# RViMLab/ECCV2022-multi-scale-and-cross-scale-contrastive-segmentation

Hardware: NVIDIA B200
Metric: ms+cs contrastive loss fwd+bwd anchor-pairs/s (higher is better)
Workload: dtype bf16

## Files before the change

### eccv2022-multi-scale-and-cross-scale-contrastive-segmentation_b200/csrc/common.cuh

```cuda
#pragma once
#include <cuda_runtime.h>
#include <cuda_bf16.h>
#include <cuda_fp16.h>
#include <stdint.h>
#include <stdio.h>
#include <stdarg.h>

#include "../../include/mscs.h"

namespace mscs {

void set_error(const char* fmt, ...);
const char* get_error();

#define MSCS_CHECK_ARG(cond, ...)                                   \
  do {                                                              \
    if (!(cond)) { ::mscs::set_error(__VA_ARGS__); return -1; }     \
  } while (0)

#define MSCS_CUDA(expr)                                                                   \
  do {                                                                                    \
    cudaError_t _e = (expr);                                                              \
    if (_e != cudaSuccess) {                                                              \
      ::mscs::set_error("%s failed: %s (%s:%d)", #expr, cudaGetErrorString(_e), __FILE__, \
// ... 31 lines not shown
  cfg.numAttrs = pdl_enabled() ? 1 : 0;
  return cudaLaunchKernelEx(&cfg, kernel, static_cast<P>(args)...);
}

__device__ __forceinline__ float warp_sum(float v) {
#pragma unroll
  for (int o = 16; o > 0; o >>= 1) v += __shfl_xor_sync(0xffffffffu, v, o);
  return v;
}

__device__ __forceinline__ float to_f32(float x) { return x; }
__device__ __forceinline__ float to_f32(__nv_bfloat16 x) { return __bfloat162float(x); }
__device__ __forceinline__ float to_f32(__half x) { return __half2float(x); }
template <typename T> __device__ __forceinline__ T from_f32(float x);
template <> __device__ __forceinline__ float from_f32<float>(float x) { return x; }
template <> __device__ __forceinline__ __nv_bfloat16 from_f32<__nv_bfloat16>(float x) { return __float2bfloat16_rn(x); }
template <> __device__ __forceinline__ __half from_f32<__half>(float x) { return __float2half_rn(x); }

__device__ __forceinline__ uint32_t pack2(__nv_bfloat16*, float a, float b) {
  const __nv_bfloat162 h = __floats2bfloat162_rn(a, b);
  return reinterpret_cast<const uint32_t&>(h);
}
__device__ __forceinline__ uint32_t pack2(__half*, float a, float b) {
  const __half2 h = __floats2half2_rn(a, b);
  return reinterpret_cast<const uint32_t&>(h);
}

__device__ __forceinline__ void st16_cs(float* p, const float (&v)[4]) {
  __stcs(reinterpret_cast<float4*>(p), make_float4(v[0], v[1], v[2], v[3]));
}
template <typename T>
__device__ __forceinline__ void st16_cs(T* p, const float (&v)[8]) {
  const uint4 u = make_uint4(pack2(p, v[0], v[1]), pack2(p, v[2], v[3]), pack2(p, v[4], v[5]), pack2(p, v[6], v[7]));
  __stcs(reinterpret_cast<uint4*>(p), u);
}

__device__ __forceinline__ void ld4(const float* p, float (&v)[4]) {
  const float4 x = *reinterpret_cast<const float4*>(p);
  v[0] = x.x; v[1] = x.y; v[2] = x.z; v[3] = x.w;
}
template <typename T>
__device__ __forceinline__ void ld4(const T* p, float (&v)[4]) {
  const uint2 u = *reinterpret_cast<const uint2*>(p);
  const T* h = reinterpret_cast<const T*>(&u);
#pragma unroll
  for (int q = 0; q < 4; ++q) v[q] = to_f32(h[q]);
}
__device__ __forceinline__ void st4_cs(float* p, const float (&v)[4]) { st16_cs(p, v); }
template <typename T>
__device__ __forceinline__ void st4_cs(T* p, const float (&v)[4]) {
  __stcs(reinterpret_cast<uint2*>(p), make_uint2(pack2(p, v[0], v[1]), pack2(p, v[2], v[3])));
}

static inline int dtype_bytes(int dtype) {
  return dtype == MSCS_DTYPE_F32 ? 4 : (dtype == MSCS_DTYPE_BF16 || dtype == MSCS_DTYPE_F16) ? 2 : 0;
}

}
```

### eccv2022-multi-scale-and-cross-scale-contrastive-segmentation_b200/csrc/gather.cu

```cuda
#include "common.cuh"

namespace mscs {

constexpr int kMaxC = 256;

__global__ void __launch_bounds__(256)
k_gather_normalize(const float* __restrict__ feat, int C, int C_pad, int plane, const int* __restrict__ pix,
                   int N, int N_pad, __nv_bfloat16* __restrict__ anc_bf16, float* __restrict__ anc_f32,
                   float* __restrict__ inv_norm) {
  pdl_trigger();
  const int lane = threadIdx.x & 31;
  const int row = blockIdx.x * (blockDim.x >> 5) + (threadIdx.x >> 5);
  if (row >= N_pad) return;
  __nv_bfloat16* orow = anc_bf16 + (size_t)row * C_pad;
  if (row >= N) {
    for (int c = lane; c < C_pad; c += 32) orow[c] = __float2bfloat16(0.f);
    return;
  }
  const int gp = pix[row];
  if (gp < 0) {
    for (int c = lane; c < C_pad; c += 32) orow[c] = __float2bfloat16(0.f);
    return;
  }
  const int b = gp / plane, p = gp - b * plane;
// ... 286 lines not shown

template <typename T>
__global__ void __launch_bounds__(256) k_scatter_rows_nhwc(const __grid_constant__ RowsBatch g) {
  int s = 0;
  while (s + 1 < g.count && (int)blockIdx.x >= g.block0[s + 1]) ++s;
  const int lane = threadIdx.x & 31;
  const int row = ((int)blockIdx.x - g.block0[s]) * 8 + (threadIdx.x >> 5);
  if (row >= g.rows[s] || (g.n_rows_dev[s] && row >= *g.n_rows_dev[s])) return;
  const int gp = g.pix[s][row];
  if (gp < 0) return;
  const int C = g.C[s];
  const float* gr = g.dF[s] + (size_t)row * g.ldF[s];
  const float* f = g.f32[s] + (size_t)row * C;
  float gv[kMaxC / 32], fv[kMaxC / 32], dot = 0.f;
#pragma unroll
  for (int q = 0; q < kMaxC / 32; ++q) {
    const int c = lane + 32 * q;
    gv[q] = (c < C) ? gr[c] : 0.f;
    fv[q] = (c < C) ? f[c] : 0.f;
    dot = fmaf(gv[q], fv[q], dot);
  }
  dot = warp_sum(dot);
  const float inv = g.inv[s][row];
  const bool clamped = inv >= 1e12f;
  T* dst = static_cast<T*>(g.dfeat[s]) + (size_t)gp * C;
#pragma unroll
  for (int q = 0; q < kMaxC / 32; ++q) {
    const int c = lane + 32 * q;
    if (c < C) dst[c] = from_f32<T>((clamped ? gv[q] : (gv[q] - fv[q] * dot)) * inv);
  }
}

template <typename T, bool GATHER>
__global__ void __launch_bounds__(256) k_rows_raw_nhwc(const __grid_constant__ RowsBatch g) {
  int s = 0;
  while (s + 1 < g.count && (int)blockIdx.x >= g.block0[s + 1]) ++s;
  const int lane = threadIdx.x & 31;
  const int row = ((int)blockIdx.x - g.block0[s]) * 8 + (threadIdx.x >> 5);
  if (row >= g.rows[s] || (g.n_rows_dev[s] && row >= *g.n_rows_dev[s])) return;
  const int gp = g.pix[s][row];
  if (gp < 0) return;
  const int C = g.C[s];
  if (GATHER) {
    const T* src = static_cast<const T*>(g.feat[s]) + (size_t)gp * C;
    float* dst = g.f32[s] + (size_t)row * C;
    for (int c = lane; c < C; c += 32) dst[c] = to_f32(__ldg(src + c));
  } else {
    const float* src = g.dF[s] + (size_t)row * g.ldF[s];
    T* dst = static_cast<T*>(g.dfeat[s]) + (size_t)gp * C;
    for (int c = lane; c < C; c += 32) dst[c] = from_f32<T>(src[c]);
  }
}

struct DenseStream {
  const float* dx[MSCS_MAX_SCALES]; const int* slot[MSCS_MAX_SCALES]; void* dfeat[MSCS_MAX_SCALES];
  int ld[MSCS_MAX_SCALES], C[MSCS_MAX_SCALES], plane[MSCS_MAX_SCALES], npix[MSCS_MAX_SCALES], blk0[MSCS_MAX_SCALES + 1];
  int count;
};
template <typename T>
__global__ void __launch_bounds__(128) k_dense_stream(const __grid_constant__ DenseStream g) {
  constexpr int P = 16 / sizeof(T);
  int s = 0;
  while (s + 1 < g.count && (int)blockIdx.x >= g.blk0[s + 1]) ++s;
  const int lin = (((int)blockIdx.x - g.blk0[s]) * 128 + (int)threadIdx.x) * P;
  if (lin >= g.npix[s]) return;
  const int plane = g.plane[s], C = g.C[s], ld = g.ld[s];
  int sl[P];
#pragma unroll
  for (int i = 0; i < P; i += 4) {
    const int4 q = *reinterpret_cast<const int4*>(g.slot[s] + lin + i);
    sl[i] = q.x; sl[i + 1] = q.y; sl[i + 2] = q.z; sl[i + 3] = q.w;
  }
  const int b = lin / plane, p = lin - b * plane;
  T* __restrict__ out = static_cast<T*>(g.dfeat[s]) + ((size_t)b * C) * plane + p;
  const float* __restrict__ dx = g.dx[s];
  const float* r[P];
  bool h[P];
#pragma unroll
  for (int i = 0; i < P; ++i) { r[i] = dx + (size_t)max(sl[i], 0) * ld; h[i] = sl[i] >= 0; }
#pragma unroll 8
  for (int c = 0; c < C; ++c) {
    float v[P];
#pragma unroll
    for (int i = 0; i < P; ++i) v[i] = h[i] ? __ldg(r[i] + c) : 0.f;
    st16_cs(out + (size_t)c * plane, v);
  }
}

}

using namespace mscs;

extern "C" int mscs_gather_normalize_sectors(const float* feat, int n, int C, int plane, const int32_t* slot, int N,
                                             void* anc_bf16, float* anc_f32, float* inv_norm, void* stream_) {
  MSCS_CHECK_ARG(feat && slot && anc_bf16 && anc_f32 && inv_norm, "null pointer argument");
  MSCS_CHECK_ARG(C >= 1 && C <= kMaxC, "C=%d unsupported (1..%d)", C, kMaxC);
  MSCS_CHECK_ARG(n >= 1 && plane >= 8 && plane % 8 == 0 && N >= 1, "bad sizes (plane must be a multiple of 8)");
  cudaStream_t st = (cudaStream_t)stream_;
  const int C_pad = (C + 63) / 64 * 64, N_pad = (N + 255) / 256 * 256;
  if (N_pad > N)
    MSCS_CUDA(cudaMemsetAsync((__nv_bfloat16*)anc_bf16 + (size_t)N * C_pad, 0,
                              sizeof(__nv_bfloat16) * (size_t)(N_pad - N) * C_pad, st));
  const int n_oct = n * (plane / 8);
  k_gather_sectors<<<ceil_div(n_oct, 8), 256, 0, st>>>(feat, C, C_pad, plane, slot, n_oct, (__nv_bfloat16*)anc_bf16,
                                                       anc_f32, inv_norm, nullptr);
  MSCS_LAUNCH_CHECK();
  return 0;
}

extern "C" int mscs_slot_map(const int32_t* pix, int N, int n_pixels, int32_t* slot, void* stream_) {
  MSCS_CHECK_ARG(pix && slot && N >= 1 && n_pixels >= 1, "bad arguments");
  cudaStream_t st = (cudaStream_t)stream_;
  MSCS_CUDA(cudaMemsetAsync(slot, 0xff, sizeof(int) * (size_t)n_pixels, st));
  k_slot_map<<<ceil_div(N, 256), 256, 0, st>>>(pix, N, slot);
  MSCS_LAUNCH_CHECK();
  return 0;
}

extern "C" int mscs_scatter_sectors_pull(void* const* slabs, int world, size_t dF_byte_off, int rows_per_rank, int ldF,
                                         const float* anc_f32, const float* inv_norm, const int32_t* slot, int n, int C,
                                         int plane, float* dfeat, void* stream_) {
  MSCS_CHECK_ARG(slabs && anc_f32 && inv_norm && slot && dfeat, "null pointer argument");
  MSCS_CHECK_ARG(world >= 1 && world <= MSCS_MAX_RANKS && rows_per_rank >= 1, "bad world %d / rows per rank %d", world,
                 rows_per_rank);
  MSCS_CHECK_ARG(C >= 1 && C <= kMaxC && ldF >= C, "C=%d / ldF=%d unsupported", C, ldF);
  MSCS_CHECK_ARG(plane % 8 == 0, "plane %d is not a multiple of 8 pixels", plane);
  PullRows pull{};
  pull.n = world; pull.rows_per_rank = rows_per_rank;
  for (int r = 0; r < world; ++r) {
    MSCS_CHECK_ARG(slabs[r] != nullptr, "peer %d: null slab pointer", r);
    pull.p[r] = reinterpret_cast<const float*>((const char*)slabs[r] + dF_byte_off);
  }
  const int n_oct = n * (plane / 8);
  k_scatter_sectors_pull<<<ceil_div(n_oct, 8), 256, 0, (cudaStream_t)stream_>>>(pull, ldF, anc_f32, inv_norm, slot,
// ... 76 lines not shown
  scatter_sectors_body(g.dF[s], g.ldF[s], g.f32[s], g.inv[s], g.slot[s], g.n_oct[s], g.C[s], g.plane[s], g.dfeat[s],
                       g.block0[s]);
}

extern "C" int mscs_scatter_sectors_batch(const mscs_scatter_item* items, int count, void* stream_) {
  MSCS_CHECK_ARG(items && count >= 1 && count <= MSCS_MAX_SCALES, "bad item count %d", count);
  ScatterBatch g{};
  g.count = count;
  int blocks = 0;
  for (int s = 0; s < count; ++s) {
    const mscs_scatter_item& it = items[s];
    MSCS_CHECK_ARG(it.dF && it.anc_f32 && it.inv_norm && it.slot && it.dfeat, "item %d: null pointer argument", s);
    MSCS_CHECK_ARG(it.C >= 1 && it.C <= kMaxC && it.ldF >= it.C, "item %d: C=%d / ldF=%d unsupported", s, it.C, it.ldF);
    MSCS_CHECK_ARG(it.plane % 8 == 0, "item %d: plane %d is not a multiple of 8 pixels", s, it.plane);
    if (int rc = check_dtype(s, it.dtype, it.dfeat, 16, "dfeat")) return rc;
    MSCS_CHECK_ARG(it.dtype == MSCS_DTYPE_F32, "item %d: the sector scatter writes fp32 gradients only", s);
    g.dF[s] = it.dF; g.f32[s] = it.anc_f32; g.inv[s] = it.inv_norm; g.slot[s] = it.slot; g.dfeat[s] = (float*)it.dfeat;
    g.ldF[s] = it.ldF; g.C[s] = it.C; g.plane[s] = it.plane; g.n_oct[s] = it.n * (it.plane / 8);
    g.block0[s] = blocks;
    blocks += ceil_div(g.n_oct[s], 8);
  }
  g.block0[count] = blocks;
  k_scatter_sectors_batch<<<blocks, 256, 0, (cudaStream_t)stream_>>>(g);
  MSCS_LAUNCH_CHECK();
  return 0;
}


extern "C" int mscs_gather_normalize(const float* feat, int n, int C, int plane, const int32_t* pix, int N,
                                     void* anc_bf16, float* anc_f32, float* inv_norm, void* stream_) {
  MSCS_CHECK_ARG(feat && pix && anc_bf16 && anc_f32 && inv_norm, "null pointer argument");
  MSCS_CHECK_ARG(C >= 1 && C <= kMaxC, "C=%d unsupported (1..%d)", C, kMaxC);
  MSCS_CHECK_ARG(n >= 1 && plane >= 1 && N >= 1, "bad sizes");
  const int C_pad = (C + 63) / 64 * 64, N_pad = (N + 255) / 256 * 256;
  k_gather_normalize<<<ceil_div(N_pad, 8), 256, 0, (cudaStream_t)stream_>>>(
      feat, C, C_pad, plane, pix, N, N_pad, (__nv_bfloat16*)anc_bf16, anc_f32, inv_norm);
  MSCS_LAUNCH_CHECK();
  return 0;
}

extern "C" int mscs_scatter_grad(const float* dF, int ldF, const float* anc_f32, const float* inv_norm,
                                 const int32_t* pix, int N, int n, int C, int plane, float* dfeat,
                                 int zero_fill, void* stream_) {
  MSCS_CHECK_ARG(dF && anc_f32 && inv_norm && pix && dfeat, "null pointer argument");
  MSCS_CHECK_ARG(C >= 1 && C <= kMaxC && ldF >= C, "C=%d / ldF=%d unsupported", C, ldF);
  cudaStream_t st = (cudaStream_t)stream_;
  if (zero_fill) MSCS_CUDA(cudaMemsetAsync(dfeat, 0, sizeof(float) * (size_t)n * C * plane, st));
  k_scatter_grad<<<ceil_div(N, 8), 256, 0, st>>>(dF, ldF, anc_f32, inv_norm, pix, N, C, plane, dfeat);
  MSCS_LAUNCH_CHECK();
  return 0;
}

template <typename T>
static int dense_stream_launch(const DenseBatch& g, const mscs_scatter_item* items, int dtype, cudaStream_t st) {
  DenseStream d{};
  int blk = 0;
  for (int s = 0; s < g.count; ++s) {
    if (items[s].dtype != dtype) continue;
    const int j = d.count++;
    d.dx[j] = g.dF[s]; d.slot[j] = g.slot[s]; d.dfeat[j] = items[s].dfeat; d.ld[j] = g.ldF[s]; d.C[j] = g.C[s];
    d.plane[j] = g.plane[s]; d.npix[j] = g.n[s] * g.plane[s]; d.blk0[j] = blk;
    blk += ceil_div(d.npix[j], 128 * (16 / (int)sizeof(T)));
  }
  if (d.count == 0) return 0;
  d.blk0[d.count] = blk;
  k_dense_stream<T><<<blk, 128, 0, st>>>(d);
  MSCS_LAUNCH_CHECK();
  return 0;
}

extern "C" int mscs_scatter_dense_batch(const mscs_scatter_item* items, const int32_t* rows, int count, void* stream_) {
  MSCS_CHECK_ARG(items && rows && count >= 1 && count <= MSCS_MAX_SCALES, "bad arguments");
  DenseBatch g{};
  g.count = count;
  int rb = 0, n_raw = 0;
  for (int s = 0; s < count; ++s) {
    const mscs_scatter_item& it = items[s];
    MSCS_CHECK_ARG(it.dF && it.slot && it.dfeat, "item %d: null pointer argument", s);
    MSCS_CHECK_ARG((it.anc_f32 == nullptr) == (it.inv_norm == nullptr),
                   "item %d: anc_f32 and inv_norm must both be set or both be NULL (raw rows)", s);
    const bool raw = it.anc_f32 == nullptr;
    n_raw += raw;
    MSCS_CHECK_ARG(it.C >= 1 && it.C <= kMaxC && it.ldF >= it.C, "item %d: C=%d / ldF=%d unsupported", s, it.C, it.ldF);
    MSCS_CHECK_ARG(it.plane % 4 == 0 && rows[s] >= 0, "item %d: plane %d is not a multiple of 4 pixels", s, it.plane);
    if (int rc = check_dtype(s, it.dtype, it.dfeat, 16, "dfeat")) return rc;
    MSCS_CHECK_ARG(it.dtype == MSCS_DTYPE_F32 || it.plane % 8 == 0,
                   "item %d: half gradients need a plane that is a multiple of 8 pixels (plane %d)", s, it.plane);
    g.dF[s] = const_cast<float*>(it.dF); g.f32[s] = it.anc_f32; g.inv[s] = it.inv_norm; g.slot[s] = it.slot;
    g.ldF[s] = it.ldF; g.C[s] = it.C; g.plane[s] = it.plane; g.n[s] = it.n; g.rows[s] = raw ? 0 : rows[s];
    g.n_rows_dev[s] = it.n_rows_dev;
    MSCS_CHECK_ARG((long long)it.n * it.C * it.plane < (1ll << 32), "item %d: more than 2^32 gradient elements", s);
    g.rowblk0[s] = rb; rb += ceil_div(g.rows[s], 8);
  }
  g.rowblk0[count] = rb;
  cudaStream_t st = (cudaStream_t)stream_;
  if (n_raw < count) {
    k_dx_rows<<<rb > 0 ? rb : 1, 256, 0, st>>>(g);
    MSCS_LAUNCH_CHECK();
  }
  if (int rc = dense_stream_launch<float>(g, items, MSCS_DTYPE_F32, st)) return rc;
  if (int rc = dense_stream_launch<__nv_bfloat16>(g, items, MSCS_DTYPE_BF16, st)) return rc;
  return dense_stream_launch<__half>(g, items, MSCS_DTYPE_F16, st);
}

enum RowsKind { kRowsGather, kRowsScatter, kRowsGatherRaw };

static int rows_check(const mscs_rows_item* items, int count, RowsKind kind) {
  MSCS_CHECK_ARG(items && count >= 1 && count <= MSCS_MAX_SCALES, "bad item count %d", count);
  const bool gather = kind != kRowsScatter;
  for (int s = 0; s < count; ++s) {
    const mscs_rows_item& it = items[s];
    if (kind == kRowsScatter) {
      MSCS_CHECK_ARG(it.pix, "item %d: null pointer argument", s);
      MSCS_CHECK_ARG((it.anc_f32 == nullptr) == (it.inv_norm == nullptr),
                     "item %d: anc_f32 and inv_norm must both be set or both be NULL (raw rows)", s);
    } else {
      MSCS_CHECK_ARG(it.pix && it.anc_f32 && (kind == kRowsGatherRaw || it.inv_norm), "item %d: null pointer argument", s);
    }
    MSCS_CHECK_ARG(it.C >= 1 && it.C <= kMaxC && it.rows >= 0, "item %d: C=%d unsupported (1..%d)", s, it.C, kMaxC);
    if (gather) MSCS_CHECK_ARG(it.feat && (kind == kRowsGatherRaw || it.anc_bf16), "item %d: null pointer argument", s);
    else MSCS_CHECK_ARG(it.dF && it.dfeat && it.ldF >= it.C, "item %d: bad gradient arguments", s);
    if (int rc = check_dtype(s, it.dtype, gather ? it.feat : it.dfeat, 1, gather ? "feat" : "dfeat")) return rc;
  }
  return 0;
}

template <typename T>
static int rows_launch(const mscs_rows_item* items, int count, RowsKind kind, bool raw, int dtype, cudaStream_t st) {
  RowsBatch g{};
  int blocks = 0;
  for (int s = 0; s < count; ++s) {
    const mscs_rows_item& it = items[s];
    if (it.dtype != dtype || (kind == kRowsScatter && (it.anc_f32 == nullptr) != raw)) continue;
    const int j = g.count++;
    g.feat[j] = it.feat; g.pix[j] = it.pix; g.n_rows_dev[j] = it.n_rows_dev;
    g.bf16[j] = (__nv_bfloat16*)it.anc_bf16; g.f32[j] = it.anc_f32; g.inv[j] = it.inv_norm;
    g.dF[j] = it.dF; g.dfeat[j] = it.dfeat; g.C[j] = it.C; g.ldF[j] = it.ldF; g.rows[j] = it.rows;
    g.block0[j] = blocks;
    blocks += ceil_div(kind == kRowsGather ? (it.rows + 255) / 256 * 256 : it.rows, 8);
  }
  g.block0[g.count] = blocks;
  if (blocks == 0) return 0;
  if (kind == kRowsGather) k_gather_rows_nhwc<T><<<blocks, 256, 0, st>>>(g);
  else if (kind == kRowsGatherRaw) k_rows_raw_nhwc<T, true><<<blocks, 256, 0, st>>>(g);
  else if (raw) k_rows_raw_nhwc<T, false><<<blocks, 256, 0, st>>>(g);
  else k_scatter_rows_nhwc<T><<<blocks, 256, 0, st>>>(g);
  MSCS_LAUNCH_CHECK();
  return 0;
}

static int rows_batch(const mscs_rows_item* items, int count, RowsKind kind, bool raw, void* stream_) {
  cudaStream_t st = (cudaStream_t)stream_;
  if (int rc = rows_launch<float>(items, count, kind, raw, MSCS_DTYPE_F32, st)) return rc;
  if (int rc = rows_launch<__nv_bfloat16>(items, count, kind, raw, MSCS_DTYPE_BF16, st)) return rc;
  return rows_launch<__half>(items, count, kind, raw, MSCS_DTYPE_F16, st);
// ... 18 lines not shown
```

### eccv2022-multi-scale-and-cross-scale-contrastive-segmentation_b200/csrc/sim_bwd.cu

```cuda
#include "sim_tc.cuh"
#include <stdlib.h>

namespace mscs {

constexpr int kBwdEpiWarps = 16;
constexpr int kBwdThreads = 128 + 32 * kBwdEpiWarps;
constexpr int kBwdStages = 3;
constexpr int kBwdSub = 64;
constexpr uint32_t kTmX = 256, kTmS = 384;

struct BwdDev {
  const int* row_cls; const int* col_seg;
  const float* row_cs; const float* row_cpn; const float* row_neg;
  const float* col_cs; const float* col_cpn; const float* col_neg;
  const __nv_bfloat16* x_rows;
  float* dF; int ld;
  int n_rows, n_cols, self_mask, y_map;
  float scale_log2, out_scale;
};
struct BwdArgs {
  alignas(64) CUtensorMap maps[MSCS_MAX_SCALES];
  BwdDev p[MSCS_MAX_PASSES];
  WorkTable work;
  const float* grad_out;
  const int* rows_dev[MSCS_MAX_PASSES]; const int* cols_dev[MSCS_MAX_PASSES];
};

__host__ __device__ constexpr size_t bwd_smem_bytes(int KB) {
  return 1024 + (size_t)(kBwdStages * KB) * kBlkBytes + (size_t)kBwdEpiWarps * 2 * 3 * 32 * sizeof(float) + 256;
}

__device__ __forceinline__ uint32_t pack_bf16(float lo, float hi) {
  __nv_bfloat162 v = __floats2bfloat162_rn(lo, hi);
  return *reinterpret_cast<uint32_t*>(&v);
}
__device__ __forceinline__ void red_add_v4(float* addr, float a, float b, float c, float d) {
  asm volatile("red.global.add.v4.f32 [%0], {%1, %2, %3, %4};" ::"l"(addr), "f"(a), "f"(b), "f"(c), "f"(d)
               : "memory");
}

template <int KB, bool DEV>
__global__ void __launch_bounds__(kBwdThreads, 1) k_sim_bwd(const __grid_constant__ BwdArgs args) {
  constexpr int CP = KB * 64;
  extern __shared__ uint8_t smem_raw[];
  uint8_t* smem = reinterpret_cast<uint8_t*>((reinterpret_cast<uintptr_t>(smem_raw) + 1023) & ~uintptr_t(1023));
  uint8_t* smB = smem;
  float* cstat = reinterpret_cast<float*>(smB + (size_t)kBwdStages * KB * kBlkBytes);
  uint64_t* bars = reinterpret_cast<uint64_t*>(cstat + kBwdEpiWarps * 2 * 3 * 32);
  uint64_t* b_full = bars;
  uint64_t* b_empty = bars + 12;
  uint64_t* s_full = bars + 15;
  uint64_t* w_full = bars + 17;
  uint64_t* df_full = bars + 19;  uint64_t* df_empty = bars + 20;
  uint64_t* x_full = bars + 21;
  uint32_t* tmem_slot = reinterpret_cast<uint32_t*>(bars + 22);

  const int warp = threadIdx.x >> 5, lane = threadIdx.x & 31;
  pdl_trigger();
  if (warp == 0 && lane == 0) {
    for (int i = 0; i < kBwdStages; ++i) {
      ptx::mbar_init(&b_full[i], 1);
      ptx::mbar_init(&b_empty[i], 1);
    }
    for (int i = 0; i < 2; ++i) { ptx::mbar_init(&s_full[i], 1); ptx::mbar_init(&w_full[i], kBwdEpiWarps); }
    ptx::mbar_init(df_full, 1); ptx::mbar_init(df_empty, kBwdEpiWarps);
    ptx::mbar_init(x_full, kBwdEpiWarps);
    ptx::fence_barrier_init();
  }
  if (warp == 2) ptx::tmem_alloc(tmem_slot, 512);
  ptx::tc_fence_before();
  __syncthreads();
  ptx::tc_fence_after();
  const uint32_t tmem_base = *tmem_slot;
  pdl_wait();
#if defined(MSCS_WAIT_PROFILE) || defined(MSCS_TRACE)
  const unsigned long long prof_t0 = ptx::globaltimer_ns();
  const long long prof_c0 = clock64();
  (void)prof_t0;
#endif
  const uint32_t tmem_dF = tmem_base;

  if (warp == 0) {
    Walker wk(args.work);
    Segment sg, nx;
    uint32_t u = 0;
    bool have = wk.next(sg);
    while (have) {
      const bool have_n = wk.next(nx);
      const BwdDev& p = args.p[sg.owner];
      for (int ct = sg.c_begin; ct < sg.c_end; ++ct, ++u) {
        const uint32_t st = u % kBwdStages, ph = (u / kBwdStages) & 1;
// ... 28 lines not shown
      ptx::umma_commit(&s_full[sb_]);
    };
    auto emit_d = [&](uint32_t cur_, uint32_t unit_, uint32_t h_, uint32_t first) {
      const uint32_t sb_ = cur_ & 1, st_ = unit_ % kBwdStages;
      const uint32_t lo1 = m_lo + ((st_ * (KB * kBlkBytes) + h_ * (kBwdSub * 128)) >> 4);
      const uint32_t w_tm = tmem_base + kTmS + sb_ * kBwdSub;
#pragma unroll
      for (int q = 0; q < 4; ++q)
        ptx::umma_ts2(tmem_dF, w_tm + q * 16, lo1 + ((q * 16 * 128) >> 4), m_hi, idesc_d, (first != 0) | (q != 0));
      if (h_ == 1) ptx::umma_commit(&b_empty[st_]);
    };
    bool have = wk.next(sg);
    while (have) {
      const bool have_n = wk.next(nx);
      ptx::mbar_wait(x_full, seg & 1, 212);
      ptx::mbar_wait(&b_full[u % kBwdStages], (u / kBwdStages) & 1, 211);
      ptx::tc_fence_after();
      MSCS_TRACE_EV(3, 0, seg);
      const uint32_t ntiles = 2 * (uint32_t)(sg.c_end - sg.c_begin);
#ifdef MSCS_TRACE
      if (blockIdx.x == 5 && lane == 0 && seg < 256u) ptx::g_trace[3 * 2048 + seg * 8 + 2] = ntiles;
      if (blockIdx.x == 5 && lane == 0 && seg == 0) ptx::g_trace[3 * 2048 + 255 * 8 + 7] = (unsigned long long)prof_c0;
#endif
      if (ptx::elect_one()) emit_s(t2, u, 0);
      __syncwarp();
      ptx::mbar_wait(df_empty, (seg & 1) ^ 1, 213);
      for (uint32_t j = 0; j < ntiles; ++j) {
        const uint32_t cur = t2 + j, sb = cur & 1, unit = u + (j >> 1), h = j & 1;
        const bool has_next = j + 1 < ntiles;
        const uint32_t unit_n = u + ((j + 1) >> 1), h_n = (j + 1) & 1;
        if (ptx::elect_one()) {
          if (has_next) {
            if (h_n == 0) {
              ptx::mbar_wait(&b_full[unit_n % kBwdStages], (unit_n / kBwdStages) & 1, 211);
              ptx::tc_fence_after();
            }
            emit_s(cur + 1, unit_n, h_n);
          }
          MSCS_TRACE_EV(0, 0, cur);
          ptx::mbar_spin_wait(&w_full[sb], (cur >> 1) & 1, 214);
          ptx::tc_fence_after();
          MSCS_TRACE_EV(0, 1, cur);
          emit_d(cur, unit, h, j);
        }
        __syncwarp();
        MSCS_TRACE_EV(0, 2, cur);
      }
      if (ptx::elect_one()) ptx::umma_commit(df_full);
      __syncwarp();
      MSCS_TRACE_EV(3, 1, seg);
      t2 += ntiles; u += ntiles >> 1; ++seg;
      sg = nx; have = have_n;
    }
  } else if (warp >= 4) {
    const int cq = (warp - 4) >> 2, quad = warp & 3;
    const int r_loc = quad * 32 + lane;
    const uint32_t lane_base = (uint32_t)(quad * 32) << 16;
    float* my_cs = cstat + (warp - 4) * (2 * 3 * 32);
    const float gout = *args.grad_out;
    Walker wk(args.work);
    Segment sg, nx;
    uint32_t t2 = 0, un = 0, seg = 0;
    bool have = wk.next(sg);
    while (have) {
      const bool have_n = wk.next(nx);
      const BwdDev& p = args.p[sg.owner];
      const int row = sg.rb * 128 + r_loc;
      int dev_rows = 0, dev_cols = 0;
      if constexpr (DEV) { dev_rows = *args.rows_dev[sg.owner]; dev_cols = *args.cols_dev[sg.owner]; }
      if (warp == 4) MSCS_TRACE_EV(3, 3, 64u + seg);
      if (cq < KB) {
        const uint4* src = reinterpret_cast<const uint4*>(p.x_rows + (size_t)row * CP + cq * 64);
        uint32_t xv[32];
#pragma unroll
        for (int i = 0; i < 8; ++i) {
          const uint4 q4 = __ldg(src + i);
          xv[4 * i] = q4.x; xv[4 * i + 1] = q4.y; xv[4 * i + 2] = q4.z; xv[4 * i + 3] = q4.w;
        }
        ptx::tmem_st32(tmem_base + lane_base + kTmX + cq * 32, xv);
        ptx::tmem_st_wait();
      }
      if (warp == 4) MSCS_TRACE_EV(3, 4, 64u + seg);
      ptx::tc_fence_before();
      __syncwarp();
      if (lane == 0) ptx::mbar_arrive(x_full);
      const bool valid = row < (DEV ? dev_rows : p.n_rows);
      int p0 = 0, p1 = 0;
      if (valid) { const int y = p.row_cls[row]; p0 = p.col_seg[y]; p1 = p.col_seg[y + 1]; }
      const unsigned plen = (unsigned)(p1 - p0);
      int wmin = valid ? p0 : 0x7fffffff, wmax = valid ? p1 : 0;
#pragma unroll
      for (int o = 16; o > 0; o >>= 1) {
        wmin = min(wmin, __shfl_xor_sync(0xffffffffu, wmin, o));
        wmax = max(wmax, __shfl_xor_sync(0xffffffffu, wmax, o));
      }
      const float rcs = (valid && p.row_cs) ? p.row_cs[row] : 0.f;
      const float rcpn = (valid && p.row_cpn) ? p.row_cpn[row] : 0.f;
      const float rneg = (valid && p.row_neg) ? p.row_neg[row] : 1.f;
      const int self_col = p.self_mask ? row : -1;
      const float scale = p.scale_log2;
      const uint64_t scale2 = ptx::pack2(scale, scale), rcs2 = ptx::pack2(rcs, rcs);
      float pf_s = 0.f, pf_pn = 0.f, pf_neg = 1.f;
      auto prefetch_cols = [&](int ct_) {
        pf_s = 0.f; pf_pn = 0.f; pf_neg = 1.f;
        if (ct_ < sg.c_end) {
          const int c = ct_ * kTileN + (lane >> 4) * kBwdSub + cq * 16 + (lane & 15);
// ... 81 lines not shown
      for (int c0 = cq * (CP / 4); c0 < (cq + 1) * (CP / 4); c0 += 16) {
        uint32_t uu[16];
        ptx::tmem_ld16(tmem_dF + lane_base + c0, uu);
        ptx::tmem_ld_wait16(uu);
        if (valid) {
#pragma unroll
          for (int c = 0; c < 16; c += 4)
            red_add_v4(drow + c0 + c, __uint_as_float(uu[c]) * sc, __uint_as_float(uu[c + 1]) * sc,
                       __uint_as_float(uu[c + 2]) * sc, __uint_as_float(uu[c + 3]) * sc);
        }
      }
      ptx::tc_fence_before();
      __syncwarp();
      if (lane == 0) ptx::mbar_arrive(df_empty);
      if (warp == 4) MSCS_TRACE_EV(3, 2, 64u + seg);
      ++seg;
      sg = nx; have = have_n;
    }
  }
  __syncwarp();
  ptx::tc_fence_before();
  __syncthreads();
  if (warp == 2) ptx::tmem_dealloc(tmem_base, 512);
#ifdef MSCS_TRACE
  if (blockIdx.x == 5 && threadIdx.x == 0) ptx::g_trace[3 * 2048 + 255 * 8 + 6] = (unsigned long long)clock64();
  if (threadIdx.x == 0 && blockIdx.x < 256) {
    ptx::g_trace[3 * 2048 + 1024 + blockIdx.x] = (unsigned long long)(clock64() - prof_c0);
    ptx::g_trace[3 * 2048 + 1280 + blockIdx.x] = prof_t0;
    ptx::g_trace[3 * 2048 + 1536 + blockIdx.x] = ptx::globaltimer_ns();
  }
#endif
#ifdef MSCS_WAIT_PROFILE
  if (blockIdx.x == 0 && threadIdx.x == 0) {
    atomicAdd(&ptx::g_wait_ns[31], ptx::globaltimer_ns() - prof_t0);
    atomicAdd(&ptx::g_wait_cnt[31], (unsigned long long)(clock64() - prof_c0));
  }
#endif
}

}

using namespace mscs;

template <int KB, bool DEV>
static int launch_bwd(const BwdArgs& args, cudaStream_t st) {
  const size_t smem = bwd_smem_bytes(KB);
  if (int rc = ensure_trap_buffer()) return rc;
  MSCS_CUDA(cudaFuncSetAttribute(k_sim_bwd<KB, DEV>, cudaFuncAttributeMaxDynamicSharedMemorySize, (int)smem));
  MSCS_CUDA(launch_k(k_sim_bwd<KB, DEV>, persistent_ctas(), kBwdThreads, smem, st, args));
  MSCS_LAUNCH_CHECK();
  return 0;
}

extern "C" int mscs_sim_backward(const mscs_sim_job* job, const float* grad_out, float* const* dF_sets,
                                 const int32_t* dF_ld, void* stream_) {
  return mscs_sim_backward_sets(job, grad_out, dF_sets, dF_ld, 0xffffffffu, stream_);
}

extern "C" int mscs_sim_backward_sets(const mscs_sim_job* job, const float* grad_out, float* const* dF_sets,
                                      const int32_t* dF_ld, uint32_t set_mask, void* stream_) {
  int rc = validate_job(job);
  if (rc) return rc;
  MSCS_CHECK_ARG(job->work && grad_out && dF_sets && dF_ld, "null pointer argument");
  const bool dev_counts = job->terms[0].n1_dev != nullptr;
  for (int t = 0; t < job->num_terms; ++t)
    MSCS_CHECK_ARG((job->terms[t].n1_dev != nullptr) == dev_counts && (job->terms[t].n2_dev != nullptr) == dev_counts,
                   "term %d: n1_dev / n2_dev must be set for every term or for none", t);
  cudaStream_t st = (cudaStream_t)stream_;
  BwdPass passes[MSCS_MAX_PASSES];
  int np = build_passes(job, passes);
  {
    int kept = 0;
    for (int i = 0; i < np; ++i)
      if ((set_mask >> passes[i].row_set) & 1u) passes[kept++] = passes[i];
    np = kept;
    if (np == 0) return 0;
  }
  size_t fwd_items = 0, ranges = 0;
  for (int t = 0; t < job->num_terms; ++t) {
    fwd_items += (size_t)ceil_div(job->terms[t].N2, 256);
    ranges += align_up(sizeof(int2) * (size_t)job->terms[t].N1, 64) +
              align_up(sizeof(int2) * (size_t)ceil_div(job->terms[t].N1, 128) * 4, 64);
  }
  char* w = (char*)job->work + 4096 + ranges +
            2 * (align_up(sizeof(WorkItem) * fwd_items, 64) + align_up(sizeof(int) * (fwd_items + 1), 64));
  BwdArgs args{};
  args.grad_out = grad_out;
  const void* bases[MSCS_MAX_SCALES]; int nmaps = 0;
  auto map_of = [&](const void* base, int rows) -> int {
    for (int i = 0; i < nmaps; ++i) if (bases[i] == base) return i;
    if (nmaps == MSCS_MAX_SCALES) return -1;
    if (make_tensor_map(&args.maps[nmaps], base, (rows + 255) / 256 * 256, job->C_pad)) return -2;
    bases[nmaps] = base;
    return nmaps++;
  };
  BuildArgs b{};
  int nitems = 0;
  for (int i = 0; i < np; ++i) {
    const BwdPass& p = passes[i];
    const int ym = map_of(p.y_bf16, p.n_cols);
    if (ym == -2) return -1;
    MSCS_CHECK_ARG(ym >= 0, "too many distinct operand matrices");
    MSCS_CHECK_ARG(dF_sets[p.row_set] && dF_ld[p.row_set] >= job->C_pad && dF_ld[p.row_set] % 4 == 0,
                   "pass %d: dF buffer of set %d missing or leading dimension < C_pad", i, p.row_set);
    args.p[i] = BwdDev{p.row_cls, p.col_seg, p.row_cs, p.row_cpn, p.row_neg, p.col_cs, p.col_cpn, p.col_neg,
                       (const __nv_bfloat16*)p.x_bf16, dF_sets[p.row_set], dF_ld[p.row_set], p.n_rows, p.n_cols,
                       p.self_mask, ym, p.scale_log2, p.out_scale};
    b.t[i] = BuildTerm{p.row_cls, p.col_seg, p.n_rows, p.n_cols, nitems, p.rb_lo, 0, 1 << 30, p.n_rows_dev, p.n_cols_dev};
    args.rows_dev[i] = p.n_rows_dev; args.cols_dev[i] = p.n_cols_dev;
    nitems += p.rb_hi - p.rb_lo;
  }
  b.num_terms = np; b.nitems = nitems; b.rows_per_item = 128; b.mode = 0;
  b.pad = 6;
  static const int pad_env = [] { const char* e = getenv("MSCS_BWD_PAD"); return e ? atoi(e) : -1; }();
  if (pad_env >= 0) b.pad = pad_env;
  b.items = (WorkItem*)w; w += align_up(sizeof(WorkItem) * (size_t)nitems, 64);
  b.prefix = (int*)w;
  rc = launch_build_work(b, st);
  if (rc) return rc;
  args.work = WorkTable{b.items, b.prefix, nitems, b.pad};
  if (dev_counts) {
    switch (job->C_pad / 64) {
      case 1: return launch_bwd<1, true>(args, st);
      case 2: return launch_bwd<2, true>(args, st);
      case 3: return launch_bwd<3, true>(args, st);
      default: return launch_bwd<4, true>(args, st);
    }
  }
  switch (job->C_pad / 64) {
    case 1: return launch_bwd<1, false>(args, st);
    case 2: return launch_bwd<2, false>(args, st);
    case 3: return launch_bwd<3, false>(args, st);
    default: return launch_bwd<4, false>(args, st);
  }
}

extern "C" int mscs_debug_wait_profile_bwd(unsigned long long* ns_out, unsigned long long* cnt_out) {
  MSCS_CUDA(cudaDeviceSynchronize());
  MSCS_CUDA(cudaMemcpyFromSymbol(ns_out, ptx::g_wait_ns, sizeof(unsigned long long) * 32));
  MSCS_CUDA(cudaMemcpyFromSymbol(cnt_out, ptx::g_wait_cnt, sizeof(unsigned long long) * 32));
  unsigned long long zero[32] = {};
  MSCS_CUDA(cudaMemcpyToSymbol(ptx::g_wait_ns, zero, sizeof(zero)));
  MSCS_CUDA(cudaMemcpyToSymbol(ptx::g_wait_cnt, zero, sizeof(zero)));
  return 0;
}

extern "C" int mscs_debug_trace_bwd(unsigned long long* out, int max_events) {
#ifdef MSCS_TRACE
  MSCS_CUDA(cudaDeviceSynchronize());
  const int n = max_events < 8192 ? max_events : 8192;
  MSCS_CUDA(cudaMemcpyFromSymbol(out, ptx::g_trace, sizeof(unsigned long long) * n));
  static unsigned long long zeros[8192];
  MSCS_CUDA(cudaMemcpyToSymbol(ptx::g_trace, zeros, sizeof(zeros)));
  return n;
#else
  (void)out; (void)max_events;
  return 0;
#endif
}
```

### eccv2022-multi-scale-and-cross-scale-contrastive-segmentation_b200/csrc/step.cu

```cuda
#include "common.cuh"
#include "../../include/mscs.h"

using namespace mscs;

namespace {

struct ChainEvents { cudaEvent_t to_sample = nullptr, to_main = nullptr; };
thread_local ChainEvents t_chain[64];

int chain_events(ChainEvents** out) {
  int dev = 0;
  MSCS_CUDA(cudaGetDevice(&dev));
  MSCS_CHECK_ARG(dev >= 0 && dev < 64, "device index %d out of range", dev);
  ChainEvents& e = t_chain[dev];
  if (!e.to_sample) {
    MSCS_CUDA(cudaEventCreateWithFlags(&e.to_sample, cudaEventDisableTiming));
    MSCS_CUDA(cudaEventCreateWithFlags(&e.to_main, cudaEventDisableTiming));
  }
  *out = &e;
  return 0;
}

inline int mark(void* ev, cudaStream_t st) {
  if (ev) MSCS_CUDA(cudaEventRecord((cudaEvent_t)ev, st));
  return 0;
}

}

#define CHAIN(call) do { if (int rc_ = (call)) return rc_; } while (0)

extern "C" int mscs_forward_chain(const mscs_forward_chain_args* a, void* sample_stream_, void* main_stream_,
                                  mscs_scale_plan* plan_host) {
  MSCS_CHECK_ARG(a && a->cfg && a->labels && a->workspace && a->plan_dev && a->job && a->gather_items,
                 "null pointer argument");
  MSCS_CHECK_ARG(a->gather_kind >= 0 && a->gather_kind <= 1, "gather_kind %d out of range", a->gather_kind);
  cudaStream_t ss = (cudaStream_t)sample_stream_, ms = (cudaStream_t)main_stream_;
  const int S = a->cfg->num_scales;
  const bool two = ss != ms;
  ChainEvents* ev = nullptr;
  if (two) {
    CHAIN(chain_events(&ev));
    MSCS_CUDA(cudaEventRecord(ev->to_sample, ms));
    MSCS_CUDA(cudaStreamWaitEvent(ss, ev->to_sample, 0));
  }
  if (a->main_zero_ptr && a->main_zero_bytes) MSCS_CUDA(cudaMemsetAsync(a->main_zero_ptr, 0, a->main_zero_bytes, ms));
  if (a->wait_event) MSCS_CUDA(cudaStreamWaitEvent(ss, (cudaEvent_t)a->wait_event, 0));
  CHAIN(mark(a->stage_events[0], ss));
  if (a->n_fill > 0) CHAIN(mscs_fill_bytes(a->fill_ptrs, a->fill_values, a->fill_bytes, a->n_fill, ss));
  if (a->labels_i16)
    CHAIN(mscs_sample_plan_i16(a->cfg, (const int16_t*)a->labels, a->workspace, a->plan_dev, ss));
  else
    CHAIN(mscs_sample_plan(a->cfg, (const int64_t*)a->labels, a->workspace, a->plan_dev, ss));
  if (plan_host) CHAIN(mscs_plan_fetch_begin(a->plan_dev, S, ss));
  CHAIN(mscs_sample_select_async(a->cfg, a->plan_dev, a->v_cap, a->workspace, a->draws, a->idx_ref, a->pair_ref, a->pix,
                                 a->cls, a->seg, a->slot, ss));
  CHAIN(mark(a->stage_events[1], ss));
  if (two) {
    MSCS_CUDA(cudaEventRecord(ev->to_main, ss));
    MSCS_CUDA(cudaStreamWaitEvent(ms, ev->to_main, 0));
  }
  CHAIN(mark(a->stage_events[2], ms));
  if (a->gather_kind == 0)
    CHAIN(mscs_gather_normalize_sectors_batch((const mscs_gather_item*)a->gather_items, S, ms));
  else
    CHAIN(mscs_gather_rows_nhwc_batch((const mscs_rows_item*)a->gather_items, S, ms));
  CHAIN(mark(a->stage_events[3], ms));
  CHAIN(mscs_sim_forward(a->job, ms));
  CHAIN(mark(a->stage_events[4], ms));
  if (!plan_host) return 0;
  return mscs_plan_fetch_end(plan_host, S);
}

extern "C" int mscs_backward_chain(const mscs_sim_job* job, const float* grad_out, float* const* dF_sets,
                                   const int32_t* dF_ld, const mscs_scatter_item* items, const int32_t* rows, int count,
                                   void* const* stage_events, void* stream_) {
  cudaStream_t st = (cudaStream_t)stream_;
  if (stage_events) CHAIN(mark(stage_events[0], st));
  CHAIN(mscs_sim_backward(job, grad_out, dF_sets, dF_ld, st));
  if (stage_events) CHAIN(mark(stage_events[1], st));
  if (count > 0) CHAIN(mscs_scatter_dense_batch(items, rows, count, st));
  if (stage_events) CHAIN(mark(stage_events[2], st));
  return 0;
}
```

Baseline: 464.4 billion.

## Zero unsampled gradient sectors inside backward kernel idle warp, scatter only sampled

Moves the zero-fill of dense feature gradients at pixels with no sampled anchor into an otherwise idle warp (warp 3) of the similarity backward kernel, so it overlaps with the matmul work. It uses evict-first streaming stores. The following dense scatter kernel then skips sector groups that are entirely unsampled and splits the channel loop across a second grid dimension for more parallelism. The cost is extra work inside the backward kernel that could lengthen its critical path, plus a sector-granularity coupling between the two kernels that must match for correctness.

```diff
diff --git a/eccv2022-multi-scale-and-cross-scale-contrastive-segmentation_b200/csrc/common.cuh b/eccv2022-multi-scale-and-cross-scale-contrastive-segmentation_b200/csrc/common.cuh
--- a/eccv2022-multi-scale-and-cross-scale-contrastive-segmentation_b200/csrc/common.cuh
+++ b/eccv2022-multi-scale-and-cross-scale-contrastive-segmentation_b200/csrc/common.cuh
@@ -107,6 +107,15 @@
   __stcs(reinterpret_cast<uint2*>(p), make_uint2(pack2(p, v[0], v[1]), pack2(p, v[2], v[3])));
 }
 
+#ifndef MSCS_SECTOR_G
+#define MSCS_SECTOR_G 2
+#endif
+constexpr int kSectorGranules = MSCS_SECTOR_G;
+int check_dense_items(const mscs_scatter_item* items, const int32_t* rows, int count);
+int scatter_dense(const mscs_scatter_item* items, const int32_t* rows, int count, bool sampled_only, cudaStream_t st);
+int sim_backward_zeroing(const mscs_sim_job* job, const float* grad_out, float* const* dF_sets, const int32_t* dF_ld,
+                         const mscs_scatter_item* items, int count, bool* zeroed, cudaStream_t st);
+
 static inline int dtype_bytes(int dtype) {
   return dtype == MSCS_DTYPE_F32 ? 4 : (dtype == MSCS_DTYPE_BF16 || dtype == MSCS_DTYPE_F16) ? 2 : 0;
 }
diff --git a/eccv2022-multi-scale-and-cross-scale-contrastive-segmentation_b200/csrc/gather.cu b/eccv2022-multi-scale-and-cross-scale-contrastive-segmentation_b200/csrc/gather.cu
--- a/eccv2022-multi-scale-and-cross-scale-contrastive-segmentation_b200/csrc/gather.cu
+++ b/eccv2022-multi-scale-and-cross-scale-contrastive-segmentation_b200/csrc/gather.cu
@@ -362,24 +362,37 @@
   }
 }
 
+#ifndef MSCS_DENSE_CHUNKS
+#define MSCS_DENSE_CHUNKS 8
+#endif
+constexpr int kDenseChunks = MSCS_DENSE_CHUNKS;
 struct DenseStream {
   const float* dx[MSCS_MAX_SCALES]; const int* slot[MSCS_MAX_SCALES]; void* dfeat[MSCS_MAX_SCALES];
   int ld[MSCS_MAX_SCALES], C[MSCS_MAX_SCALES], plane[MSCS_MAX_SCALES], npix[MSCS_MAX_SCALES], blk0[MSCS_MAX_SCALES + 1];
   int count;
 };
-template <typename T>
+template <typename T, bool SAMPLED>
 __global__ void __launch_bounds__(128) k_dense_stream(const __grid_constant__ DenseStream g) {
   constexpr int P = 16 / sizeof(T);
   int s = 0;
   while (s + 1 < g.count && (int)blockIdx.x >= g.blk0[s + 1]) ++s;
   const int lin = (((int)blockIdx.x - g.blk0[s]) * 128 + (int)threadIdx.x) * P;
-  if (lin >= g.npix[s]) return;
+  const bool in = lin < g.npix[s];
+  if (!SAMPLED && !in) return;
   const int plane = g.plane[s], C = g.C[s], ld = g.ld[s];
   int sl[P];
 #pragma unroll
   for (int i = 0; i < P; i += 4) {
-    const int4 q = *reinterpret_cast<const int4*>(g.slot[s] + lin + i);
+    const int4 q = (SAMPLED && !in) ? make_int4(-1, -1, -1, -1) : *reinterpret_cast<const int4*>(g.slot[s] + lin + i);
     sl[i] = q.x; sl[i + 1] = q.y; sl[i + 2] = q.z; sl[i + 3] = q.w;
+  }
+  if (SAMPLED) {
+    int all_neg = -1;
+#pragma unroll
+    for (int i = 0; i < P; ++i) all_neg &= sl[i];
+#pragma unroll
+    for (int o = 1; o < kSectorGranules; o <<= 1) all_neg &= __shfl_xor_sync(0xffffffffu, all_neg, o);
+    if (!in || all_neg < 0) return;
   }
   const int b = lin / plane, p = lin - b * plane;
   T* __restrict__ out = static_cast<T*>(g.dfeat[s]) + ((size_t)b * C) * plane + p;
@@ -388,8 +401,10 @@
   bool h[P];
 #pragma unroll
   for (int i = 0; i < P; ++i) { r[i] = dx + (size_t)max(sl[i], 0) * ld; h[i] = sl[i] >= 0; }
+  const int cper = SAMPLED ? (C + kDenseChunks - 1) / kDenseChunks : C;
+  const int c_lo = SAMPLED ? (int)blockIdx.y * cper : 0, c_hi = SAMPLED ? min(C, c_lo + cper) : C;
 #pragma unroll 8
-  for (int c = 0; c < C; ++c) {
+  for (int c = c_lo; c < c_hi; ++c) {
     float v[P];
 #pragma unroll
     for (int i = 0; i < P; ++i) v[i] = h[i] ? __ldg(r[i] + c) : 0.f;
@@ -572,7 +587,8 @@
 }
 
 template <typename T>
-static int dense_stream_launch(const DenseBatch& g, const mscs_scatter_item* items, int dtype, cudaStream_t st) {
+static int dense_stream_launch(const DenseBatch& g, const mscs_scatter_item* items, int dtype, bool sampled_only,
+                               cudaStream_t st) {
   DenseStream d{};
   int blk = 0;
   for (int s = 0; s < g.count; ++s) {
@@ -584,14 +600,15 @@
   }
   if (d.count == 0) return 0;
   d.blk0[d.count] = blk;
-  k_dense_stream<T><<<blk, 128, 0, st>>>(d);
-  MSCS_LAUNCH_CHECK();
-  return 0;
-}
-
-extern "C" int mscs_scatter_dense_batch(const mscs_scatter_item* items, const int32_t* rows, int count, void* stream_) {
+  if (sampled_only) k_dense_stream<T, true><<<dim3(blk, kDenseChunks), 128, 0, st>>>(d);
+  else k_dense_stream<T, false><<<blk, 128, 0, st>>>(d);
+  MSCS_LAUNCH_CHECK();
+  return 0;
+}
+
+static int dense_batch(const mscs_scatter_item* items, const int32_t* rows, int count, DenseBatch& g, int* n_raw_out) {
   MSCS_CHECK_ARG(items && rows && count >= 1 && count <= MSCS_MAX_SCALES, "bad arguments");
-  DenseBatch g{};
+  g = DenseBatch{};
   g.count = count;
   int rb = 0, n_raw = 0;
   for (int s = 0; s < count; ++s) {
@@ -613,14 +630,33 @@
     g.rowblk0[s] = rb; rb += ceil_div(g.rows[s], 8);
   }
   g.rowblk0[count] = rb;
-  cudaStream_t st = (cudaStream_t)stream_;
+  *n_raw_out = n_raw;
+  return 0;
+}
+
+int mscs::check_dense_items(const mscs_scatter_item* items, const int32_t* rows, int count) {
+  DenseBatch g;
+  int n_raw = 0;
+  return dense_batch(items, rows, count, g, &n_raw);
+}
+
+int mscs::scatter_dense(const mscs_scatter_item* items, const int32_t* rows, int count, bool sampled_only,
+                        cudaStream_t st) {
+  DenseBatch g;
+  int n_raw = 0;
+  if (int rc = dense_batch(items, rows, count, g, &n_raw)) return rc;
   if (n_raw < count) {
+    const int rb = g.rowblk0[count];
     k_dx_rows<<<rb > 0 ? rb : 1, 256, 0, st>>>(g);
     MSCS_LAUNCH_CHECK();
   }
-  if (int rc = dense_stream_launch<float>(g, items, MSCS_DTYPE_F32, st)) return rc;
-  if (int rc = dense_stream_launch<__nv_bfloat16>(g, items, MSCS_DTYPE_BF16, st)) return rc;
-  return dense_stream_launch<__half>(g, items, MSCS_DTYPE_F16, st);
+  if (int rc = dense_stream_launch<float>(g, items, MSCS_DTYPE_F32, sampled_only, st)) return rc;
+  if (int rc = dense_stream_launch<__nv_bfloat16>(g, items, MSCS_DTYPE_BF16, sampled_only, st)) return rc;
+  return dense_stream_launch<__half>(g, items, MSCS_DTYPE_F16, sampled_only, st);
+}
+
+extern "C" int mscs_scatter_dense_batch(const mscs_scatter_item* items, const int32_t* rows, int count, void* stream_) {
+  return scatter_dense(items, rows, count, false, (cudaStream_t)stream_);
 }
 
 enum RowsKind { kRowsGather, kRowsScatter, kRowsGatherRaw };
diff --git a/eccv2022-multi-scale-and-cross-scale-contrastive-segmentation_b200/csrc/sim_bwd.cu b/eccv2022-multi-scale-and-cross-scale-contrastive-segmentation_b200/csrc/sim_bwd.cu
--- a/eccv2022-multi-scale-and-cross-scale-contrastive-segmentation_b200/csrc/sim_bwd.cu
+++ b/eccv2022-multi-scale-and-cross-scale-contrastive-segmentation_b200/csrc/sim_bwd.cu
@@ -18,12 +18,19 @@
   int n_rows, n_cols, self_mask, y_map;
   float scale_log2, out_scale;
 };
+struct ZeroJob {
+  const int* slot[MSCS_MAX_SCALES]; char* dfeat[MSCS_MAX_SCALES];
+  int C[MSCS_MAX_SCALES], plane[MSCS_MAX_SCALES], npix[MSCS_MAX_SCALES], esize[MSCS_MAX_SCALES];
+  int u0[MSCS_MAX_SCALES + 1];
+  int count;
+};
 struct BwdArgs {
   alignas(64) CUtensorMap maps[MSCS_MAX_SCALES];
   BwdDev p[MSCS_MAX_PASSES];
   WorkTable work;
   const float* grad_out;
   const int* rows_dev[MSCS_MAX_PASSES]; const int* cols_dev[MSCS_MAX_PASSES];
+  ZeroJob zero;
 };
 
 __host__ __device__ constexpr size_t bwd_smem_bytes(int KB) {
@@ -37,6 +44,58 @@
 __device__ __forceinline__ void red_add_v4(float* addr, float a, float b, float c, float d) {
   asm volatile("red.global.add.v4.f32 [%0], {%1, %2, %3, %4};" ::"l"(addr), "f"(a), "f"(b), "f"(c), "f"(d)
                : "memory");
+}
+
+__device__ __forceinline__ void st_zero16_evict_first(char* p, uint64_t pol) {
+  asm volatile("st.global.L1::no_allocate.L2::cache_hint.v4.b32 [%0], {%1, %1, %1, %1}, %2;" ::"l"(p), "r"(0), "l"(pol)
+               : "memory");
+}
+
+__device__ __noinline__ void zero_unsampled_sectors(const ZeroJob& z, int lane) {
+  constexpr int G = kSectorGranules;
+  uint64_t pol;
+  asm volatile("createpolicy.fractional.L2::evict_first.b64 %0, 1.0;" : "=l"(pol));
+  const int total = z.u0[z.count];
+  const int lo = (int)((long long)total * blockIdx.x / gridDim.x);
+  const int hi = (int)((long long)total * (blockIdx.x + 1) / gridDim.x);
+  for (int s = 0; s < z.count; ++s) {
+    const int ua = max(lo, z.u0[s]) - z.u0[s], ub = min(hi, z.u0[s + 1]) - z.u0[s];
+    if (ua >= ub) continue;
+    const int C = z.C[s], plane = z.plane[s], npix = z.npix[s], es = z.esize[s], P = 16 / es;
+    const size_t pstride = (size_t)plane * es;
+    int strip = ua / C, c = ua - strip * C;
+    for (int u = ua; u < ub; ++strip, c = 0) {
+      const int cend = min(C, c + (ub - u));
+      u += cend - c;
+      const int q0 = (strip * 32 + lane) * G * P;
+      int all_neg = -1;
+      for (int i = 0; i < G * P; i += 4)
+        if (q0 + i < npix) {
+          const int4 v = __ldg(reinterpret_cast<const int4*>(z.slot[s] + q0 + i));
+          all_neg &= v.x & v.y & v.z & v.w;
+        }
+      char* gp[G];
+      bool zg[G];
+      bool any = false;
+#pragma unroll
+      for (int i = 0; i < G; ++i) {
+        const int j = 32 * i + lane;
+        const int q = (strip * 32 * G + j) * P, img = q / plane;
+        zg[i] = __shfl_sync(0xffffffffu, all_neg, j / G) < 0 && q < npix;
+        gp[i] = z.dfeat[s] + ((size_t)img * C * plane + (q - img * plane)) * es + c * pstride;
+        any |= zg[i];
+      }
+      if (!__any_sync(0xffffffffu, any)) continue;
+#pragma unroll 2
+      for (int k = c; k < cend; ++k) {
+#pragma unroll
+        for (int i = 0; i < G; ++i) {
+          if (zg[i]) st_zero16_evict_first(gp[i], pol);
+          gp[i] += pstride;
+        }
+      }
+    }
+  }
 }
 
 template <int KB, bool DEV>
@@ -171,6 +230,8 @@
       t2 += ntiles; u += ntiles >> 1; ++seg;
       sg = nx; have = have_n;
     }
+  } else if (warp == 3) {
+    if (args.zero.count) zero_unsampled_sectors(args.zero, lane);
   } else if (warp >= 4) {
     const int cq = (warp - 4) >> 2, quad = warp & 3;
     const int r_loc = quad * 32 + lane;
@@ -358,13 +419,9 @@
   return 0;
 }
 
-extern "C" int mscs_sim_backward(const mscs_sim_job* job, const float* grad_out, float* const* dF_sets,
-                                 const int32_t* dF_ld, void* stream_) {
-  return mscs_sim_backward_sets(job, grad_out, dF_sets, dF_ld, 0xffffffffu, stream_);
-}
-
-extern "C" int mscs_sim_backward_sets(const mscs_sim_job* job, const float* grad_out, float* const* dF_sets,
-                                      const int32_t* dF_ld, uint32_t set_mask, void* stream_) {
+static int sim_backward(const mscs_sim_job* job, const float* grad_out, float* const* dF_sets, const int32_t* dF_ld,
+                        uint32_t set_mask, const ZeroJob* zero, bool* zeroed, cudaStream_t st) {
+  if (zeroed) *zeroed = false;
   int rc = validate_job(job);
   if (rc) return rc;
   MSCS_CHECK_ARG(job->work && grad_out && dF_sets && dF_ld, "null pointer argument");
@@ -372,7 +429,6 @@
   for (int t = 0; t < job->num_terms; ++t)
     MSCS_CHECK_ARG((job->terms[t].n1_dev != nullptr) == dev_counts && (job->terms[t].n2_dev != nullptr) == dev_counts,
                    "term %d: n1_dev / n2_dev must be set for every term or for none", t);
-  cudaStream_t st = (cudaStream_t)stream_;
   BwdPass passes[MSCS_MAX_PASSES];
   int np = build_passes(job, passes);
   {
@@ -392,6 +448,7 @@
             2 * (align_up(sizeof(WorkItem) * fwd_items, 64) + align_up(sizeof(int) * (fwd_items + 1), 64));
   BwdArgs args{};
   args.grad_out = grad_out;
+  if (zero) args.zero = *zero;
   const void* bases[MSCS_MAX_SCALES]; int nmaps = 0;
   auto map_of = [&](const void* base, int rows) -> int {
     for (int i = 0; i < nmaps; ++i) if (bases[i] == base) return i;
@@ -425,6 +482,7 @@
   rc = launch_build_work(b, st);
   if (rc) return rc;
   args.work = WorkTable{b.items, b.prefix, nitems, b.pad};
+  if (zeroed) *zeroed = zero != nullptr;
   if (dev_counts) {
     switch (job->C_pad / 64) {
       case 1: return launch_bwd<1, true>(args, st);
@@ -439,6 +497,31 @@
     case 3: return launch_bwd<3, false>(args, st);
     default: return launch_bwd<4, false>(args, st);
   }
+}
+
+extern "C" int mscs_sim_backward(const mscs_sim_job* job, const float* grad_out, float* const* dF_sets,
+                                 const int32_t* dF_ld, void* stream_) {
+  return sim_backward(job, grad_out, dF_sets, dF_ld, 0xffffffffu, nullptr, nullptr, (cudaStream_t)stream_);
+}
+
+extern "C" int mscs_sim_backward_sets(const mscs_sim_job* job, const float* grad_out, float* const* dF_sets,
+                                      const int32_t* dF_ld, uint32_t set_mask, void* stream_) {
+  return sim_backward(job, grad_out, dF_sets, dF_ld, set_mask, nullptr, nullptr, (cudaStream_t)stream_);
+}
+
+int mscs::sim_backward_zeroing(const mscs_sim_job* job, const float* grad_out, float* const* dF_sets,
+                               const int32_t* dF_ld, const mscs_scatter_item* items, int count, bool* zeroed,
+                               cudaStream_t st) {
+  ZeroJob z{};
+  z.count = count;
+  for (int s = 0; s < count; ++s) {
+    const mscs_scatter_item& it = items[s];
+    const int es = dtype_bytes(it.dtype), P = 16 / es;
+    z.slot[s] = it.slot; z.dfeat[s] = (char*)it.dfeat; z.C[s] = it.C; z.plane[s] = it.plane; z.esize[s] = es;
+    z.npix[s] = it.n * it.plane;
+    z.u0[s + 1] = z.u0[s] + ceil_div(z.npix[s], 32 * kSectorGranules * P) * it.C;
+  }
+  return sim_backward(job, grad_out, dF_sets, dF_ld, 0xffffffffu, &z, zeroed, st);
 }
 
 extern "C" int mscs_debug_wait_profile_bwd(unsigned long long* ns_out, unsigned long long* cnt_out) {
diff --git a/eccv2022-multi-scale-and-cross-scale-contrastive-segmentation_b200/csrc/step.cu b/eccv2022-multi-scale-and-cross-scale-contrastive-segmentation_b200/csrc/step.cu
--- a/eccv2022-multi-scale-and-cross-scale-contrastive-segmentation_b200/csrc/step.cu
+++ b/eccv2022-multi-scale-and-cross-scale-contrastive-segmentation_b200/csrc/step.cu
@@ -76,10 +76,18 @@
                                    const int32_t* dF_ld, const mscs_scatter_item* items, const int32_t* rows, int count,
                                    void* const* stage_events, void* stream_) {
   cudaStream_t st = (cudaStream_t)stream_;
+  bool zeroed = false;
+  if (count > 0) CHAIN(check_dense_items(items, rows, count));
   if (stage_events) CHAIN(mark(stage_events[0], st));
-  CHAIN(mscs_sim_backward(job, grad_out, dF_sets, dF_ld, st));
+#ifdef MSCS_ZERO_OFF
+  if (false)
+#else
+  if (count > 0)
+#endif
+    CHAIN(sim_backward_zeroing(job, grad_out, dF_sets, dF_ld, items, count, &zeroed, st));
+  else CHAIN(mscs_sim_backward(job, grad_out, dF_sets, dF_ld, st));
   if (stage_events) CHAIN(mark(stage_events[1], st));
-  if (count > 0) CHAIN(mscs_scatter_dense_batch(items, rows, count, st));
+  if (count > 0) CHAIN(scatter_dense(items, rows, count, zeroed, st));
   if (stage_events) CHAIN(mark(stage_events[2], st));
   return 0;
 }
```

Result: faster. 485.2 billion, median of 6 (+4.5%).
